# casys-kaist/CoVA

Hardware: AMD Instinct MI355X
Metric: compressed-domain frames/sec (BlobNet+bboxcc) at 1080p b=256 (higher is better)
Workload: dtype f16

## Files before the change

cova_amd/csrc/bboxcc.hip:

```cpp
#include <algorithm>
#include <cstdint>
#include <mutex>
#include <vector>

#include "bboxcc_body.h"
#include "bboxcc_wave.h"
#include "covahip_dev.h"
#include "internal.h"

namespace {

using namespace ccbody;

__global__ __launch_bounds__(CC_THREADS) void bboxcc_kernel(const uint8_t *__restrict__ masks, CcGeom g, ccwave::WvGeom wg,
                                                             int area_thresh, covahip_box *__restrict__ boxes,
                                                             int32_t *__restrict__ counts, int max_boxes,
                                                             const int32_t *__restrict__ list,
                                                             const int32_t *__restrict__ n_list,
                                                             const int32_t *__restrict__ stat_src, int32_t *__restrict__ stat_dst,
                                                             int stat_batch, int stat_cap) {
    extern __shared__ __attribute__((aligned(16))) uint8_t smem[];
    if (stat_dst && blockIdx.x == 0 && threadIdx.x < 8)
        stat_dst[threadIdx.x] = threadIdx.x < 5 ? stat_src[threadIdx.x] : threadIdx.x == 5 ? stat_batch : threadIdx.x == 6 ? stat_cap : 0;
    auto one = [&](int frame) {
// ... 32 lines not shown
                                                                    int area_thresh, covahip_box *__restrict__ boxes,
                                                                    int32_t *__restrict__ counts, int max_boxes,
                                                                    const int32_t *__restrict__ list, const int32_t *__restrict__ n_list,
                                                                    int32_t *__restrict__ ovf_list, int32_t *__restrict__ ovf_n,
                                                                    int base_cap, int32_t *__restrict__ n_big,
                                                                    int32_t *__restrict__ zero_next) {
    extern __shared__ __attribute__((aligned(16))) uint8_t smem[];
    const int lane = threadIdx.x & 63, wave = threadIdx.x >> 6;
    uint8_t *const sm = smem + (size_t)wave * g.wave_bytes;
    if constexpr (!LIST) {
        if (zero_next && blockIdx.x == 0 && threadIdx.x < 8) zero_next[threadIdx.x] = 0;
        const int frame = blockIdx.x * WV_WAVES + wave;
        if (frame >= batch) return;
        const int n = ccwave::frame_wave(masks + (size_t)frame * g.H * g.W, sm, g, area_thresh, boxes + (size_t)frame * max_boxes,
                                         counts + frame, max_boxes, lane);
        if (lane == 0) {
            if (n > g.cap) {
                const int k = atomicAdd(ovf_n, 1);
                if (k < batch) ovf_list[k] = frame;
            }
            if (n_big && (frame & 15) == 0 && n > base_cap)
                atomicAdd(n_big + (n > 2 * base_cap ? 2 : 2 * n > 3 * base_cap ? 1 : 0), 1);
        }
    } else {
        const int nl = min(*n_list, batch);
        for (int k = blockIdx.x * WV_WAVES + wave; k < nl; k += gridDim.x * WV_WAVES) {
            const int frame = list[k];
            const int n = ccwave::frame_wave(masks + (size_t)frame * g.H * g.W, sm, g, area_thresh, boxes + (size_t)frame * max_boxes,
                                             counts + frame, max_boxes, lane);
            if (lane == 0 && n > g.cap) {
                const int k2 = atomicAdd(ovf_n, 1);
                if (k2 < batch) ovf_list[k2] = frame;
            }
            ccwave::wave_fence();
        }
    }
}

template <typename K>
int open_lds(covahip_ctx *ctx, K kernel, size_t lds) {
    if (lds <= 64 * 1024) return COVAHIP_OK;
    static std::mutex mu;
    static std::vector<std::pair<int, const void *>> opened;
    const void *fn = reinterpret_cast<const void *>(kernel);
    std::lock_guard<std::mutex> lock(mu);
    for (auto &o : opened)
        if (o.first == ctx->device && o.second == fn) return COVAHIP_OK;
    COVAHIP_CHECK_HIP(ctx, hipFuncSetAttribute(fn, hipFuncAttributeMaxDynamicSharedMemorySize, 160 * 1024 - 64));
    opened.emplace_back(ctx->device, fn);
    return COVAHIP_OK;
}

}

constexpr int WAVE_CAP = 128;
int covahip_bboxcc_launch(covahip_ctx *ctx, const uint8_t *d_mask, int batch, int h, int w, int area_thresh,
                          covahip_box *d_boxes, int32_t *d_counts, int max_boxes) {
    if (batch == 0) return COVAHIP_OK;
    CtxLane &ln = ctx->lane();
    CcGeom g;
    const size_t lds = cc_plan(h, w, g);
    const int num_cu = ctx->props.multiProcessorCount;
    ccwave::WvGeom wg;
    const int nb = ((h + 1) / 2) * ((w + 1) / 2);
    int cap = ctx->cc_wave_cap;
    if (cap == 0) {
        cap = -1;
        if (batch > 3 * num_cu) {
            if (ln.cc_stat && ln.cc_stat[5] > 0) {
                const int64_t c1 = 16 * (int64_t)ln.cc_stat[2], c2 = 16 * (int64_t)ln.cc_stat[3], c3 = 16 * (int64_t)ln.cc_stat[4], sb = ln.cc_stat[5];
                ln.cc_first_cap = 4 * c3 > sb ? 4 * WAVE_CAP : 4 * (c2 + c3) > sb ? 2 * WAVE_CAP : 4 * (c1 + c2 + c3) > sb ? 3 * WAVE_CAP / 2 : WAVE_CAP;
            }
            cap = ln.cc_first_cap ? ln.cc_first_cap : WAVE_CAP;
        }
    }
    cap = std::min(cap, nb);
    const bool aligned = (reinterpret_cast<uintptr_t>(d_mask) & 7) == 0 && (((size_t)h * w) & 7) == 0;
    ccwave::WvGeom wfull{};
    size_t lds_wg = lds;
    if (ctx->cc_wave_cap >= 0 && aligned && ccwave::wv_plan(h, w, nb, wfull) && (size_t)wfull.wave_bytes <= 160 * 1024 - 256)
        lds_wg = (size_t)wfull.wave_bytes;
    else
        wfull.cap = 0;
    if (cap > 0 && aligned && ccwave::wv_plan(h, w, cap, wg) &&
        (size_t)WV_WAVES * wg.wave_bytes <= 160 * 1024 - 64 && (cap >= nb || lds_wg)) {
        const bool can_overflow = cap < nb;
        ccwave::WvGeom wg2{};
        const int cap2 = std::min(4 * cap, nb);
        const bool second = can_overflow && cap2 > cap && ccwave::wv_plan(h, w, cap2, wg2) &&
                            (size_t)WV_WAVES * wg2.wave_bytes <= 160 * 1024 - 64;
        const bool third = can_overflow && (!second || cap2 < nb);
        int32_t *ovf = nullptr;
        if (can_overflow) {
            const size_t need = (2 * (size_t)batch + 16) * sizeof(int32_t);
            const bool fresh = need > ln.cc_ovf_bytes;
            int rc = covahip_ensure_buffer(ctx, &ln.cc_ovf, &ln.cc_ovf_bytes, need);
            if (rc) return rc;
            if (fresh) {
                COVAHIP_CHECK_HIP(ctx, hipMemsetAsync(ln.cc_ovf, 0, 16 * sizeof(int32_t), ctx->stream));
                ln.cc_stat_turn = 0;
            }
            ovf = (int32_t *)ln.cc_ovf;
            if (!ln.cc_stat_ring) {
                COVAHIP_CHECK_HIP(ctx, hipHostMalloc((void **)&ln.cc_stat_ring, 8 * sizeof(int32_t), hipHostMallocMapped));
                for (int k = 0; k < 8; k++) ln.cc_stat_ring[k] = 0;
                ln.cc_stat = ln.cc_stat_ring;
            }
        }
        const unsigned set = can_overflow ? (ln.cc_stat_turn & 1) : 0;
        int32_t *cnt = ovf ? ovf + 8 * set : nullptr, *cnt_next = ovf ? ovf + 8 * (set ^ 1) : nullptr;
        int32_t *n1 = cnt, *n2 = cnt ? cnt + 1 : nullptr, *n_big = cnt ? cnt + 2 : nullptr;
        int32_t *list1 = ovf ? ovf + 16 : nullptr, *list2 = ovf ? ovf + 16 + batch : nullptr;
        const bool second_now = second && !(ln.cc_stat && ln.cc_stat[5] > 0 && ln.cc_stat[0] == 0);
        const size_t wlds = (size_t)WV_WAVES * wg.wave_bytes;
        int rc = open_lds(ctx, bboxcc_wave_kernel<false>, wlds);
        if (rc) return rc;
        if (second) rc = open_lds(ctx, bboxcc_wave_kernel<true>, (size_t)WV_WAVES * wg2.wave_bytes);
        if (rc) return rc;
        {
            ProfScope ps(ctx, "bboxcc_wave_kernel");
            hipLaunchKernelGGL(bboxcc_wave_kernel<false>, dim3((batch + WV_WAVES - 1) / WV_WAVES), dim3(WV_WAVES * 64), wlds, ctx->stream,
                               d_mask, wg, batch, area_thresh, d_boxes, d_counts, max_boxes, (const int32_t *)nullptr,
                               (const int32_t *)nullptr, list1, n1, WAVE_CAP, n_big, cnt_next);
            COVAHIP_CHECK_HIP(ctx, hipGetLastError());
            if (can_overflow) ln.cc_stat_turn++;
        }
        if (second_now) {
            const size_t wlds2 = (size_t)WV_WAVES * wg2.wave_bytes;
            const int per_cu = std::max(1, (int)((160 * 1024 - 256) / wlds2));
            const int grid = std::min((batch + WV_WAVES - 1) / WV_WAVES, per_cu * num_cu);
            ProfScope ps(ctx, "bboxcc_wave_kernel_2");
            hipLaunchKernelGGL(bboxcc_wave_kernel<true>, dim3(grid), dim3(WV_WAVES * 64), wlds2, ctx->stream, d_mask, wg2, batch, area_thresh,
                               d_boxes, d_counts, max_boxes, (const int32_t *)list1, (const int32_t *)n1, list2, n2, 0, (int32_t *)nullptr,
                               (int32_t *)nullptr);
            COVAHIP_CHECK_HIP(ctx, hipGetLastError());
        }
        if (can_overflow) {
            rc = open_lds(ctx, bboxcc_kernel, lds_wg);
            if (rc) return rc;
            int32_t *stat_dev = nullptr;
            COVAHIP_CHECK_HIP(ctx, hipHostGetDevicePointer((void **)&stat_dev, ln.cc_stat_ring, 0));
            const bool have_list = third || !second_now;
            const bool quiet = ln.cc_stat && ln.cc_stat[5] > 0 && ln.cc_stat[0] == 0;
            ProfScope ps(ctx, "bboxcc_kernel");
            hipLaunchKernelGGL(bboxcc_kernel, dim3(!have_list ? 1 : quiet ? 32 : std::min(batch, 2 * num_cu)), dim3(CC_THREADS), lds_wg, ctx->stream, d_mask, g, wfull,
                               area_thresh, d_boxes, d_counts, max_boxes, (const int32_t *)(second_now ? list2 : list1),
                               (const int32_t *)(second_now ? n2 : n1), (const int32_t *)cnt, stat_dev, batch, cap);
            COVAHIP_CHECK_HIP(ctx, hipGetLastError());
            ln.cc_stat_batch = batch;
            ln.cc_stat_cap = cap;
            ln.cc_second_skipped = !second_now;
        } else {
            ln.cc_stat_batch = 0;
        }
        return COVAHIP_OK;
    }
    ln.cc_stat_batch = 0;
    if (!lds_wg) {
        CcGeom gb;
        const size_t slab = cc_plan_global(h, w, gb);
        if (!slab) return COVAHIP_ERR_UNSUPPORTED;
        const int grid = std::min(batch, 2 * num_cu);
        int rc = covahip_ensure_buffer(ctx, &ln.cc_slab, &ln.cc_slab_bytes, slab * grid);
        if (rc) return rc;
        ProfScope ps(ctx, "bboxcc_big_kernel");
        hipLaunchKernelGGL(bboxcc_big_kernel, dim3(grid), dim3(CC_THREADS), 0, ctx->stream, d_mask, gb, (uint8_t *)ln.cc_slab, slab,
// ... 63 lines not shown
```

cova_amd/csrc/bboxcc_wave.h:

```cpp
#pragma once
#include <cstdint>

#include "bboxcc_body.h"

#ifdef PHASE_TIMING
__device__ unsigned long long g_ccph[8];
#define CCWG_MARK(i)                                                        \
    do {                                                                    \
        if (tid == 0) {                                                     \
            const unsigned long long now_ = __builtin_amdgcn_s_memrealtime(); \
            atomicAdd(&g_ccph[i], now_ - cc_last_);                         \
            cc_last_ = now_;                                                \
        }                                                                   \
    } while (0)
#else
#define CCWG_MARK(i) do { } while (0)
#endif

namespace ccwave {

struct WvGeom {
    int H, W, BH, BW, NXB;
    int cap;
    int rows_bytes;
    int wave_bytes;
    uint32_t mNXB;
};

inline bool wv_plan(int h, int w, int cap, WvGeom &g) {
    if (h <= 0 || w <= 0 || h > 128 || w > 128 || (w & 7) || cap <= 0) return false;
    g.H = h; g.W = w;
    g.BH = (h + 1) / 2; g.BW = (w + 1) / 2;
    g.NXB = w / 8;
    g.cap = cap;
    g.rows_bytes = (2 * g.BH + 2) * 16;
    g.wave_bytes = g.rows_bytes + cap * 24;
    g.mNXB = g.NXB <= 1 ? 0u : (uint32_t)(((1ull << 32) / (uint32_t)g.NXB) + 1);
    return true;
}

__device__ __forceinline__ uint32_t nz_bits(uint32_t x) {
    return (((x & 0x7F7F7F7Fu) + 0x7F7F7F7Fu) | x) & 0x80808080u;
}
__device__ __forceinline__ void wave_fence() {
    __builtin_amdgcn_fence(__ATOMIC_RELEASE, "wavefront");
    __builtin_amdgcn_wave_barrier();
    __builtin_amdgcn_fence(__ATOMIC_ACQUIRE, "wavefront");
}
__device__ __forceinline__ int ctz64(uint64_t x) { return __ffsll((unsigned long long)x) - 1; }
__device__ __forceinline__ int nth_set_bit64(uint64_t x, int k) {
    uint32_t w = (uint32_t)x;
    int pos = 0;
    int c = __popc(w);
    if (k >= c) { k -= c; w = (uint32_t)(x >> 32); pos = 32; }
    c = __popc(w & 0xFFFFu);
    if (k >= c) { k -= c; w >>= 16; pos += 16; }
    c = __popc(w & 0xFFu);
    if (k >= c) { k -= c; w >>= 8; pos += 8; }
    c = __popc(w & 0xFu);
    if (k >= c) { k -= c; w >>= 4; pos += 4; }
    w &= 0xFu;
    for (int i = 0; i < k; i++) w &= w - 1;
    return pos + (__ffs((int)w) - 1);
}
__device__ __forceinline__ uint64_t mask_upto(int e) { return e >= 63 ? ~0ull : ((2ull << e) - 1); }

__device__ __forceinline__ int frame_wave(const uint8_t *m, uint8_t *sm, const WvGeom &g, int area_thresh, covahip_box *ob,
                                           int32_t *count_out, int max_boxes, int lane) {
    uint32_t *rows = reinterpret_cast<uint32_t *>(sm);
    uint32_t *lab = reinterpret_cast<uint32_t *>(sm + g.rows_bytes);
    uint32_t *s_area = lab + g.cap, *s_minx = s_area + g.cap, *s_maxx = s_minx + g.cap, *s_miny = s_maxx + g.cap,
             *s_maxy = s_miny + g.cap;

    for (int i = lane; i < g.rows_bytes / 4; i += 64) rows[i] = 0;
    wave_fence();
    const int npieces = g.H * g.NXB;
    constexpr int UN = 8;
    for (int q0 = lane; q0 < npieces; q0 += 64 * UN) {
        uint2 v[UN];
#pragma unroll
        for (int k = 0; k < UN; k++) {
            const int q = q0 + 64 * k;
            v[k] = q < npieces ? *reinterpret_cast<const uint2 *>(m + (size_t)q * 8) : make_uint2(0, 0);
        }
#pragma unroll
        for (int k = 0; k < UN; k++) {
            if ((v[k].x | v[k].y) == 0) continue;
            const int q = q0 + 64 * k;
            const int y = g.mNXB ? (int)__umulhi((uint32_t)q, g.mNXB) : q, xc = q - y * g.NXB;
            const uint32_t tl = nz_bits(v[k].x), th = nz_bits(v[k].y);
            const uint32_t e = (((tl & 0x00800080u) * 0x00800100u) >> 30) | ((((th & 0x00800080u) * 0x00800100u) >> 30) << 2);
            const uint32_t o = (((tl & 0x80008000u) * 0x00008001u) >> 30) | ((((th & 0x80008000u) * 0x00008001u) >> 30) << 2);
            uint32_t *rw = rows + (y + 1) * 4 + (xc >> 3);
            const int sh = 4 * (xc & 7);
            if (e) atomicOr(rw, e << sh);
            if (o) atomicOr(rw + 2, o << sh);
        }
    }

    wave_fence();
    uint64_t a = 0, b = 0, c = 0, d = 0, ue = 0, uo = 0;
    if (lane < g.BH) {
        const uint4 ru = reinterpret_cast<const uint4 *>(rows)[2 * lane];
        const uint4 r0 = reinterpret_cast<const uint4 *>(rows)[2 * lane + 1];
        const uint4 r1 = reinterpret_cast<const uint4 *>(rows)[2 * lane + 2];
        ue = ru.x | ((uint64_t)ru.y << 32); uo = ru.z | ((uint64_t)ru.w << 32);
        a = r0.x | ((uint64_t)r0.y << 32);  b = r0.z | ((uint64_t)r0.w << 32);
        c = r1.x | ((uint64_t)r1.y << 32);  d = r1.z | ((uint64_t)r1.w << 32);
    }
    const uint64_t F = a | b | c | d;
    const uint64_t J = (a | c) & ((b | d) << 1);
    const uint64_t S = F & ~J;
// ... 77 lines not shown
    wave_fence();
    int total = 0;
    for (int i0 = 0; i0 < n; i0 += 64) {
        const int i = i0 + lane;
        const bool keep = i < n && lab[i] == (uint32_t)i && (int)s_area[i] >= area_thresh;
        const uint64_t bal = __ballot(keep);
        if (keep) {
            const int pos = total + __popcll((unsigned long long)(bal & ((1ull << lane) - 1)));
            if (pos < max_boxes) {
                covahip_box bx;
                bx.left = (int32_t)s_minx[i];
                bx.top = (int32_t)s_miny[i];
                bx.width = (int32_t)(s_maxx[i] - s_minx[i] + 1);
                bx.height = (int32_t)(s_maxy[i] - s_miny[i] + 1);
                bx.area_px = (int32_t)s_area[i];
                ob[pos] = bx;
            }
        }
        total += __popcll((unsigned long long)bal);
    }
    if (lane == 0) *count_out = total;
    return n;
}

template <int NTH, bool PLANES = false>
__device__ __forceinline__ void frame_wg(const uint8_t *m, uint8_t *sm, const WvGeom &g, int area_thresh, covahip_box *ob,
                                         int32_t *count_out, int max_boxes, int tid, uint32_t *planes = nullptr) {
    constexpr int NWV = NTH / 64;
    const int lane = tid & 63, wave = tid >> 6;
    uint32_t *rows = PLANES ? planes : reinterpret_cast<uint32_t *>(sm);
    uint32_t *lab = reinterpret_cast<uint32_t *>(sm + g.rows_bytes);
    uint32_t *s_area = lab + g.cap, *s_minx = s_area + g.cap, *s_maxx = s_minx + g.cap, *s_miny = s_maxx + g.cap,
             *s_maxy = s_miny + g.cap;
    __shared__ uint32_t wave_tot[NWV];
#ifdef PHASE_TIMING
    unsigned long long cc_last_ = __builtin_amdgcn_s_memrealtime();
#endif

    if constexpr (!PLANES) {
    for (int i = tid; i < g.rows_bytes / 4; i += NTH) rows[i] = 0;
    __syncthreads();
    const int npieces = g.H * g.NXB;
    for (int q = tid; q < npieces; q += NTH) {
        const uint2 v = *reinterpret_cast<const uint2 *>(__builtin_assume_aligned(m + (size_t)q * 8, 8));
        if ((v.x | v.y) == 0) continue;
        const int y = g.mNXB ? (int)__umulhi((uint32_t)q, g.mNXB) : q, xc = q - y * g.NXB;
        const uint32_t tl = nz_bits(v.x), th = nz_bits(v.y);
        const uint32_t e = (((tl & 0x00800080u) * 0x00800100u) >> 30) | ((((th & 0x00800080u) * 0x00800100u) >> 30) << 2);
        const uint32_t o = (((tl & 0x80008000u) * 0x00008001u) >> 30) | ((((th & 0x80008000u) * 0x00008001u) >> 30) << 2);
        uint32_t *rw = rows + (y + 1) * 4 + (xc >> 3);
        const int sh = 4 * (xc & 7);
        if (e) atomicOr(rw, e << sh);
        if (o) atomicOr(rw + 2, o << sh);
    }
    __syncthreads();
    }
    CCWG_MARK(0);
    uint64_t a = 0, b = 0, c = 0, d = 0, ue = 0, uo = 0;
    if (lane < g.BH) {
        const uint4 ru = reinterpret_cast<const uint4 *>(rows)[2 * lane];
        const uint4 r0 = reinterpret_cast<const uint4 *>(rows)[2 * lane + 1];
        const uint4 r1 = reinterpret_cast<const uint4 *>(rows)[2 * lane + 2];
        ue = ru.x | ((uint64_t)ru.y << 32); uo = ru.z | ((uint64_t)ru.w << 32);
        a = r0.x | ((uint64_t)r0.y << 32);  b = r0.z | ((uint64_t)r0.w << 32);
        c = r1.x | ((uint64_t)r1.y << 32);  d = r1.z | ((uint64_t)r1.w << 32);
    }
    const uint64_t F = a | b | c | d;
    const uint64_t J = (a | c) & ((b | d) << 1);
    const uint64_t S = F & ~J;
    const uint64_t cU = (a | b) & (ue | uo), cUL = a & (uo << 1), cUR = b & (ue >> 1);
    const int nr = __popcll((unsigned long long)S);
    int incl = nr;
#pragma unroll
    for (int o = 1; o < 64; o <<= 1) {
        const int t = __shfl_up(incl, o, 64);
        if (lane >= o) incl += t;
    }
    const int base = incl - nr;
    const int n = __shfl(incl, 63, 64);
    uint64_t S_up = (uint64_t)__shfl_up((unsigned long long)S, 1, 64), J_up = (uint64_t)__shfl_up((unsigned long long)J, 1, 64);
    int base_up = __shfl_up(base, 1, 64);
    if (lane == 0) { S_up = 0; J_up = 0; base_up = 0; }
    for (int i = tid; i < n; i += NTH) lab[i] = (uint32_t)i;
    __syncthreads();
    CCWG_MARK(1);
    for (int k = wave; __any(k < nr); k += NWV) {
        uint64_t Tu = 0;
        const int idx = base + k;
        if (k < nr) {
            const int s = nth_set_bit64(S, k);
            const uint64_t jr = (J >> s) >> 1;
            const int e = s + (~jr ? ctz64(~jr) : 0);
            const uint64_t mk = mask_upto(e) & ~((1ull << s) - 1);
            const uint64_t ra = a & mk, rb = b & mk, rc = c & mk, rd = d & mk;
            s_area[idx] = (uint32_t)(__popcll((unsigned long long)ra) + __popcll((unsigned long long)rb) +
                                     __popcll((unsigned long long)rc) + __popcll((unsigned long long)rd));
            s_minx[idx] = (uint32_t)(2 * s + (((a | c) >> s) & 1 ? 0 : 1));
            s_maxx[idx] = (uint32_t)(2 * e + (((b | d) >> e) & 1 ? 1 : 0));
            s_miny[idx] = (uint32_t)(2 * lane + ((ra | rb) ? 0 : 1));
            s_maxy[idx] = (uint32_t)(2 * lane + ((rc | rd) ? 1 : 0));
            Tu = (cU & mk) | ((cUL & mk) >> 1) | ((cUR & mk) << 1);
        }
        while (__any(Tu != 0)) {
            if (Tu) {
                const int p = ctz64(Tu);
                const int rank = __popcll((unsigned long long)(S_up << (63 - p))) - 1;
                const uint64_t jr = (J_up >> p) >> 1;
                const int e_up = p + (~jr ? ctz64(~jr) : 0);
                Tu &= ~mask_upto(e_up);
                ccbody::uf_union(lab, (uint32_t)idx, (uint32_t)(base_up + rank));
            }
        }
    }
    __syncthreads();
    CCWG_MARK(2);
    for (int i = tid; i < n; i += NTH) {
        const uint32_t root = ccbody::uf_find(lab, (uint32_t)i);
        if (root != (uint32_t)i) {
            lab[i] = root;
            atomicAdd(&s_area[root], s_area[i]);
            atomicMin(&s_minx[root], s_minx[i]);
            atomicMax(&s_maxx[root], s_maxx[i]);
            atomicMin(&s_miny[root], s_miny[i]);
            atomicMax(&s_maxy[root], s_maxy[i]);
        }
    }
    __syncthreads();
    CCWG_MARK(3);
    const int per = (n + NTH - 1) / NTH;
    const int i0 = tid * per;
    uint32_t cnt = 0;
    for (int k = 0; k < per; k++) {
        const int i = i0 + k;
        if (i < n && lab[i] == (uint32_t)i && (int)s_area[i] >= area_thresh) cnt++;
    }
    uint32_t inc2 = cnt;
#pragma unroll
    for (int o = 1; o < 64; o <<= 1) {
        const uint32_t t = __shfl_up(inc2, o, 64);
        if (lane >= o) inc2 += t;
    }
    if (lane == 63) wave_tot[wave] = inc2;
    __syncthreads();
    uint32_t pbase = 0, total = 0;
#pragma unroll
    for (int k = 0; k < NWV; k++) {
        const uint32_t t = wave_tot[k];
        if (k < wave) pbase += t;
        total += t;
    }
    uint32_t pos = pbase + inc2 - cnt;
    for (int k = 0; k < per; k++) {
        const int i = i0 + k;
        if (i < n && lab[i] == (uint32_t)i && (int)s_area[i] >= area_thresh) {
            if ((int)pos < max_boxes) {
                covahip_box bx;
                bx.left = (int32_t)s_minx[i];
                bx.top = (int32_t)s_miny[i];
                bx.width = (int32_t)(s_maxx[i] - s_minx[i] + 1);
                bx.height = (int32_t)(s_maxy[i] - s_miny[i] + 1);
                bx.area_px = (int32_t)s_area[i];
                ob[pos] = bx;
            }
            pos++;
        }
    }
    if (tid == 0) *count_out = (int32_t)total;
    __syncthreads();
// ... 5 lines not shown
```

cova_amd/csrc/blobnet.hip:

```cpp
#include <algorithm>
#include <cstdlib>
#include <cstring>
#include <vector>

#include "blobnet.h"
#include "covahip_dev.h"

namespace {

constexpr uint32_t W_MAGIC = 0x57485643;
constexpr size_t N_PARAMS = 320305;

}

static void free_model(covahip_ctx *ctx, covahip_blobnet *m) {
    if (!m) return;
    blobnet_release_mfma(ctx, m);
    for (BnWorkspace &ws : m->ws) {
        for (int i = 0; i <= BN_LEVELS; i++)
            if (ws.act[i]) hipFree(ws.act[i]);
        for (int j = 0; j < BN_LEVELS; j++)
            if (ws.dact[j]) hipFree(ws.dact[j]);
        if (ws.pbuf) hipFree(ws.pbuf);
        if (ws.part) hipFree(ws.part);
// ... 240 lines not shown
    BnInput plan;
    plan.dry = true;
    for (int pass = 0; pass < (n_models > 1 ? 8 : 4) && !rc; pass++) {
        const int b = (pass & 1) ? max_batch : 1;
        plan.n_frames = (pass & 2) ? b + BN_T - 1 : 0;
        plan.mixed = (pass & 4) != 0;
        rc = blobnet_forward_mfma(ctx, m, m->ws[0], plan, b, nullptr, nullptr, nullptr, nullptr);
    }
    return rc;
}

extern "C" {

static const float *check_blob(const void *weights, size_t weights_bytes) {
    if (!weights || weights_bytes < 64) return nullptr;
    uint32_t hdr[16];
    std::memcpy(hdr, weights, 64);
    static const uint32_t want[] = {W_MAGIC, 1, 4, 3, 16, 32, 64, 128, 64, 32, 16, 16, (uint32_t)N_PARAMS};
    for (int i = 0; i < 13; i++)
        if (hdr[i] != want[i]) return nullptr;
    if (weights_bytes != 64 + N_PARAMS * sizeof(float)) return nullptr;
    return reinterpret_cast<const float *>(static_cast<const uint8_t *>(weights) + 64);
}

int covahip_blobnet_load(covahip_ctx *ctx, const void *weights, size_t weights_bytes, int h_mb, int w_mb, int t,
                         int max_batch) {
    if (!ctx || !weights) return COVAHIP_ERR_INVALID_ARG;
    if (t == BN_T && h_mb >= 16 && w_mb >= 16 && h_mb <= 1024 && w_mb <= 1024 && max_batch > 0 && !check_blob(weights, weights_bytes))
        return COVAHIP_ERR_BAD_WEIGHTS;
    return covahip_blobnet_load_set(ctx, 1, &weights, &weights_bytes, h_mb, w_mb, t, max_batch);
}

int covahip_blobnet_load_set(covahip_ctx *ctx, int n_models, const void *const *weights, const size_t *weights_bytes, int h_mb,
                             int w_mb, int t, int max_batch) {
    if (!ctx || !weights || !weights_bytes || h_mb <= 0 || w_mb <= 0 || max_batch <= 0) return COVAHIP_ERR_INVALID_ARG;
    if (n_models < 1 || n_models > COVAHIP_MAX_MODELS) return COVAHIP_ERR_INVALID_ARG;
    for (int k = 0; k < n_models; k++)
        if (!weights[k]) return COVAHIP_ERR_INVALID_ARG;
    if (t != BN_T) return COVAHIP_ERR_UNSUPPORTED;
    if (h_mb < 16 || w_mb < 16 || h_mb > 1024 || w_mb > 1024) return COVAHIP_ERR_UNSUPPORTED;
    std::vector<const float *> h_w(n_models);
    bool bad = false;
    for (int k = 0; k < n_models; k++) bad = bad || !(h_w[k] = check_blob(weights[k], weights_bytes[k]));

    COVAHIP_CHECK_HIP(ctx, hipSetDevice(ctx->device));
    covahip_blobnet_destroy(ctx);
    if (bad) return COVAHIP_ERR_BAD_WEIGHTS;
    covahip_blobnet *m = new covahip_blobnet();
    int rc = build_model(ctx, m, h_w.data(), n_models, h_mb, w_mb, max_batch);
    if (rc == COVAHIP_OK && hipStreamSynchronize(ctx->stream) != hipSuccess) rc = COVAHIP_ERR_HIP;
    if (rc) {
        hipStreamSynchronize(ctx->stream);
        (void)hipGetLastError();
        free_model(ctx, m);
        return rc;
    }
    ctx->blobnet = m;
    return COVAHIP_OK;
}

int covahip_blobnet_num_models(covahip_ctx *ctx, int *n_models) {
    if (!ctx || !n_models) return COVAHIP_ERR_INVALID_ARG;
    if (!ctx->blobnet) return COVAHIP_ERR_NOT_LOADED;
    *n_models = ctx->blobnet->n_models;
    return COVAHIP_OK;
}

int covahip_blobnet_macs_per_frame(covahip_ctx *ctx, int64_t *macs) {
    if (!ctx || !macs) return COVAHIP_ERR_INVALID_ARG;
    if (!ctx->blobnet) return COVAHIP_ERR_NOT_LOADED;
    *macs = ctx->blobnet->macs_per_frame;
    return COVAHIP_OK;
}

int covahip_blobnet_set_enc_plan(covahip_ctx *ctx, int level, int nbands, int nbuf) {
    if (!ctx || level < 1 || level > 3 || nbands < 0 || nbands > 64 || (nbands && nbuf != 1 && nbuf != 2)) return COVAHIP_ERR_INVALID_ARG;
    ctx->enc_plan[level].nbands = nbands;
    ctx->enc_plan[level].nbuf = nbands ? nbuf : 0;
    return COVAHIP_OK;
}

int covahip_blobnet_set_impl(covahip_ctx *ctx, int impl) {
    if (!ctx || !ctx->blobnet) return COVAHIP_ERR_NOT_LOADED;
    if (impl != 1 && (impl < 4 || impl > 10)) return COVAHIP_ERR_INVALID_ARG;
    ctx->blobnet->fuse_dec = impl != 4;
    ctx->blobnet->enc1_tile16 = impl != 5;
    ctx->blobnet->enc_rowtiles = impl != 6;
    ctx->blobnet->fuse_enc23 = impl == 7 ? 0 : impl == 8 ? 2 : 1;
    ctx->blobnet->tail_part = impl != 9;
    ctx->blobnet->tail_rows = impl != 10;
    return COVAHIP_OK;
}

static int filter_placed(covahip_ctx *ctx, covahip_blobnet *m, const uint8_t *d_src, int n_frames, const int32_t *stack_index,
                         int batch, int area_thresh, covahip_box *d_boxes, int32_t *d_counts, int max_boxes, float *d_logits,
                         uint8_t *d_mask, bool packed = false, const uint8_t *model_ids = nullptr) {
    if (!d_mask) {
        CtxLane &l = ctx->lane();
        int rc = covahip_ensure_buffer(ctx, &l.cc_scratch, &l.cc_scratch_bytes, (size_t)batch * m->H * m->W);
        if (rc) return rc;
        d_mask = (uint8_t *)l.cc_scratch;
    }
    BnInput in;
    if (n_frames > 0) {
        int rc = prepare_frames(ctx, m, m->ws[ctx->cur_lane], d_src, n_frames, stack_index, batch, in, model_ids);
        if (rc) return rc;
        in.packed = packed;
    } else {
        in.stack = d_src;
    }
    return filter_dev(ctx, in, batch, d_logits, d_mask, true, area_thresh, d_boxes, d_counts, max_boxes, n_frames > 0 ? nullptr : model_ids);
}

static int filter_any(covahip_ctx *ctx, const uint8_t *src, int n_frames, const int32_t *stack_index, int batch,
                      int area_thresh, covahip_box *boxes, int32_t *counts, int max_boxes, float *logits, uint8_t *mask,
                      int mem_kind, const uint8_t *model_ids = nullptr) {
    if (!ctx || batch < 0 || max_boxes < 0 || n_frames < 0) return COVAHIP_ERR_INVALID_ARG;
    covahip_blobnet *m = ctx->blobnet;
    if (!m) return COVAHIP_ERR_NOT_LOADED;
    if (batch == 0) return COVAHIP_OK;
    if (!src || !counts || (!boxes && max_boxes > 0) || batch > m->max_batch) return COVAHIP_ERR_INVALID_ARG;
    if (int rc = check_model_ids(m, model_ids, batch)) return rc;
    COVAHIP_CHECK_HIP(ctx, hipSetDevice(ctx->device));
    const bool by_frames = n_frames > 0;
    const size_t hw = (size_t)m->H * m->W;
    const size_t in_bytes = by_frames ? (size_t)n_frames * hw * 4 : (size_t)batch * BN_T * hw * 4;
    const size_t mask_bytes = (size_t)batch * hw;
    const size_t logit_bytes = mask_bytes * sizeof(float);
    const size_t box_bytes = (size_t)batch * max_boxes * sizeof(covahip_box);
    const size_t cnt_bytes = (size_t)batch * sizeof(int32_t);
    auto al = [](size_t x) { return (x + 255) & ~(size_t)255; };
    if (mem_kind != COVAHIP_MEM_DEVICE && mem_kind != COVAHIP_MEM_HOST) return COVAHIP_ERR_INVALID_ARG;

    if (mem_kind == COVAHIP_MEM_DEVICE) {
        LaneScope lane(ctx);
        if (!lane.ok()) return COVAHIP_ERR_HIP;
        return filter_placed(ctx, m, src, n_frames, stack_index, batch, area_thresh, boxes, counts, max_boxes, logits, mask, false, model_ids);
    }
    if (int rc = covahip_primary_op(ctx)) return rc;
    const uint8_t *d_src = src;
    int rc = covahip_ensure_buffer(ctx, &ctx->stage_in, &ctx->stage_in_bytes, in_bytes);
    if (rc) return rc;
    rc = covahip_ensure_buffer(ctx, &ctx->stage_out, &ctx->stage_out_bytes,
                               al(mask_bytes) + al(logit_bytes) + al(box_bytes) + al(cnt_bytes));
    if (rc) return rc;
    uint8_t *base = (uint8_t *)ctx->stage_out;
    uint8_t *d_mask = base;
    float *d_logits = logits ? (float *)(base + al(mask_bytes)) : nullptr;
    covahip_box *d_boxes = (covahip_box *)(base + al(mask_bytes) + al(logit_bytes));
    int32_t *d_counts = (int32_t *)(base + al(mask_bytes) + al(logit_bytes) + al(box_bytes));
    COVAHIP_CHECK_HIP(ctx, hipMemcpyAsync(ctx->stage_in, src, in_bytes, hipMemcpyHostToDevice, ctx->stream));
    d_src = (const uint8_t *)ctx->stage_in;
    rc = filter_placed(ctx, m, d_src, n_frames, stack_index, batch, area_thresh, d_boxes, d_counts, max_boxes, d_logits, d_mask, false,
                       model_ids);
    if (rc) return rc;
    if (logits) COVAHIP_CHECK_HIP(ctx, hipMemcpyAsync(logits, d_logits, logit_bytes, hipMemcpyDeviceToHost, ctx->stream));
    if (mask) COVAHIP_CHECK_HIP(ctx, hipMemcpyAsync(mask, d_mask, mask_bytes, hipMemcpyDeviceToHost, ctx->stream));
    if (box_bytes) COVAHIP_CHECK_HIP(ctx, hipMemcpyAsync(boxes, d_boxes, box_bytes, hipMemcpyDeviceToHost, ctx->stream));
    COVAHIP_CHECK_HIP(ctx, hipMemcpyAsync(counts, d_counts, cnt_bytes, hipMemcpyDeviceToHost, ctx->stream));
    COVAHIP_CHECK_HIP(ctx, hipStreamSynchronize(ctx->stream));
    return COVAHIP_OK;
}

int covahip_filter_forward(covahip_ctx *ctx, const uint8_t *rgba_stack, int batch, int area_thresh,
                           covahip_box *boxes, int32_t *counts, int max_boxes, float *logits, uint8_t *mask,
                           int mem_kind) {
    return filter_any(ctx, rgba_stack, 0, nullptr, batch, area_thresh, boxes, counts, max_boxes, logits, mask, mem_kind);
}

int covahip_filter_forward_m(covahip_ctx *ctx, const uint8_t *rgba_stack, const uint8_t *model_ids, int batch, int area_thresh,
                             covahip_box *boxes, int32_t *counts, int max_boxes, float *logits, uint8_t *mask, int mem_kind) {
    return filter_any(ctx, rgba_stack, 0, nullptr, batch, area_thresh, boxes, counts, max_boxes, logits, mask, mem_kind, model_ids);
}
// ... 169 lines not shown
```

cova_amd/csrc/blobnet_mfma.hip:

```cpp
#include <algorithm>
#include <cmath>
#include <cstdlib>
#include <cstring>
#include <mutex>
#include <type_traits>
#include <utility>
#include <vector>

#include "bboxcc_body.h"
#include "bboxcc_wave.h"
#include "blobnet.h"

typedef _Float16 half8 __attribute__((ext_vector_type(8)));
typedef _Float16 half4 __attribute__((ext_vector_type(4)));
typedef float f32x16 __attribute__((ext_vector_type(16)));
typedef float f32x4 __attribute__((ext_vector_type(4)));
typedef _Float16 half2v __attribute__((ext_vector_type(2)));

namespace {

constexpr float BN_EPS = 1e-3f;
constexpr int WG = 256;

struct EncPrep {
// ... 2688 lines not shown
    return true;
}

struct DecPlan {
    DecArgs a;
    DecMs am;
    BnLevelGeom in, out;
    bool half;
    int ci, GH, grid;
    size_t row_bytes, lds;
};
int plan_dec_block(const Fwd &f, int j, DecPlan &p) {
    const covahip_blobnet *m = f.m;
    const Prepared *pr = f.pr;
    const BnLevelGeom in = m->lv[BN_LEVELS - j], out = m->lv[BN_LEVELS - 1 - j];
    const bool last = j == BN_LEVELS - 1;
    const bool half = last && f.part_written;
    const int ci_j = half ? m->dec_ci[j] / 2 : m->dec_ci[j];
    DecArgs &a = p.a;
    a.up = j == 0 ? nullptr : f.ws.dact[j - 1];
    a.skip = f.ws.act[BN_LEVELS - j];
    a.out = last ? nullptr : f.ws.dact[j];
    a.logits = last ? f.d_logits : nullptr;
    a.mask = last ? f.d_mask : nullptr;
    a.wfrag = (const half8 *)(f.prep + (half ? pr->final_w_up : last ? pr->final_w : pr->dec[j].wfrag));
    a.part = half ? f.ws.part : nullptr;
    a.epi = (const float *)(f.prep + (last ? pr->final_epi : pr->dec[j].epi));
    a.B = f.batch; a.Hi = in.H; a.Wi = in.W; a.Hd = out.H; a.Wd = out.W; a.cy = m->dec_cy[j]; a.cx = m->dec_cx[j];
    a.Ts = j == 0 ? 1 : BN_T;
    p.am = DecMs{f.inp.model_ids, f.mstride};
    const int GH = in.H + 1;
    const size_t row_bytes = (size_t)(in.W + 2) * ci_j * 2;
    const size_t wbytes = (size_t)(last ? 1 : 4 * m->dec_co[j] / 32) * (4 * ci_j / 16) * 1024;
    const bool heavy = wbytes >= 192 * 1024 && (size_t)(GH + 1) * row_bytes <= 72 * 1024;
    int nbands = 1;
    if (!heavy)
        while (nbands < GH && (((size_t)((GH + nbands - 1) / nbands) + 1) * row_bytes > 30 * 1024 ||
                               (long long)f.batch * nbands < 2LL * f.num_cu))
            nbands++;
    a.nbands = nbands; a.mNb = magic(nbands); a.mGW = magic(in.W + 1);
    a.mRC = magic((in.W + 2) * (ci_j / 8)); a.zero = f.prep + pr->zero;
    a.swz = choose_swz(false, ci_j, in.W, 0, (GH + nbands - 1) / nbands);
    const size_t tile_bytes = (((size_t)((GH + nbands - 1) / nbands) + 1) * row_bytes + 15) & ~(size_t)15;
    const size_t mask_bytes = last ? ((((size_t)2 * ((GH + nbands - 1) / nbands) * out.W) + 15) & ~(size_t)15) : 0;
    const size_t scr_bytes = last ? 0 : (size_t)std::max(4, 4 * m->dec_co[j] / 32) * 2048;
    p.lds = tile_bytes + mask_bytes + scr_bytes;
    a.mask_off = (int)tile_bytes;
    a.scr_off = (int)tile_bytes;
    if (p.lds > 160 * 1024 - 256) return COVAHIP_ERR_UNSUPPORTED;
    p.in = in; p.out = out; p.half = half; p.ci = ci_j; p.GH = GH; p.row_bytes = row_bytes;
    p.grid = std::min(f.batch * nbands, (heavy ? 1 : 4) * f.num_cu);
    return COVAHIP_OK;
}
int launch_dec_block(const Fwd &f, int j, const DecPlan &p) {
    if (j == 0)
        return launched(f, with_bools([&](auto MS) {
            return launch(f, "dec0_mfma", dec_mfma<0, 128, 64, false, MS.value>, p.grid, 512, p.lds, p.a, p.am);
        }, f.ms));
    if (j == 1)
        return launched(f, with_bools([&](auto MS) {
            return launch(f, "dec1_mfma", dec_mfma<64, 64, 32, false, MS.value>, p.grid, 256, p.lds, p.a, p.am);
        }, f.ms));
    if (j == 2)
        return launched(f, with_bools([&](auto MS) {
            return launch(f, "dec2_mfma", dec_mfma<32, 32, 16, false, MS.value>, p.grid, 256, p.lds, p.a, p.am);
        }, f.ms));
    return launched(f, with_bools([&](auto HALF, auto MS) {
        return launch(f, "dec3_final_mfma", dec_mfma<16, HALF.value ? 0 : 16, 16, true, MS.value>, p.grid, 256, p.lds, p.a, p.am);
    }, p.half, f.ms));
}
int run_dec_block(const Fwd &f, int j) {
    DecPlan p;
    if (int rc = plan_dec_block(f, j, p)) return rc;
    return launch_dec_block(f, j, p);
}

bool run_tail_fused(const Fwd &f, const DecPlan &p) {
    const BnLevelGeom in = p.in, out = p.out;
    const int GH = p.GH;
    Dec3ccArgs t;
    size_t cc_bytes = ccbody::cc_plan(out.H, out.W, t.g);
    t.use_wv = f.ctx->cc_wave_cap >= 0 && ccwave::wv_plan(out.H, out.W, ((out.H + 1) / 2) * ((out.W + 1) / 2), t.wg) ? 1 : 0;
    if (t.use_wv) cc_bytes = (size_t)t.wg.wave_bytes;
    if (!cc_bytes) return false;
    const size_t mfull = ((size_t)out.H * out.W + 15) & ~(size_t)15;
    const size_t partb = p.half ? (size_t)GH * (in.W + 1) * 16 : 0;
    int best_nb = 0;
    long long best_cost = -1;
    for (int nb = 1; nb <= GH; nb++) {
        const size_t tb = (((size_t)((GH + nb - 1) / nb) + 1) * p.row_bytes + 15) & ~(size_t)15;
        const size_t nbuf = nb == 1 ? 1 : 2;
        if (std::max(nbuf * tb, cc_bytes) + mfull + partb > 160 * 1024 - 512) continue;
        long long rounds = 0;
        for (int k = 0; k < nb; k++) {
            const int nu = (k + 1) * GH / nb - k * GH / nb;
            rounds += ((nu * (in.W + 1) + 31) / 32 + 15) / 16;
        }
        const long long cost = rounds * 8 + nb;
        if (best_cost < 0 || cost < best_cost) { best_cost = cost; best_nb = nb; }
    }
    if (!best_nb) return false;
    const size_t tb = (((size_t)((GH + best_nb - 1) / best_nb) + 1) * p.row_bytes + 15) & ~(size_t)15;
    t.d = p.a;
    t.ms = p.am;
    t.d.nbands = best_nb; t.d.mNb = magic(best_nb);
    t.d.swz = choose_swz(false, p.ci, in.W, 0, (GH + best_nb - 1) / best_nb);
    t.boxes = f.cc->boxes; t.counts = f.cc->counts;
    t.area_thresh = f.cc->area_thresh; t.max_boxes = f.cc->max_boxes;
    t.tile_bytes = (int)tb; t.cc_off = 0;
    t.mfull_off = (int)std::max((best_nb == 1 ? 1 : 2) * tb, cc_bytes);
    t.part_off = (int)((size_t)t.mfull_off + mfull);
    const size_t tl = (size_t)t.part_off + partb;
    const int grid = std::min(f.batch, 2 * f.num_cu);
    if (p.half && t.use_wv && best_nb == 1 && in.W + 1 <= 64 && f.m->tail_rows && (out.W & 7) == 0 &&
        (size_t)t.wg.rows_bytes <= mfull && (!f.d_mask || (reinterpret_cast<uintptr_t>(f.d_mask) & 3) == 0)) {
        t.d.swz = Swz{3, 1, 0, 0, 0};
        t.d.mRC = magic(out.W / 4);
        return !with_bools([&](auto MS) {
            return launch(f, "dec3_bboxcc_fused", dec3cc_rows_mfma<MS.value>, grid, ccbody::CC_THREADS, tl, t);
        }, f.ms);
    }
    return !with_bools([&](auto WV, auto PART, auto MS) {
        return launch(f, "dec3_bboxcc_fused", dec3cc_mfma<WV.value, PART.value, MS.value>, grid, ccbody::CC_THREADS, tl, t);
    }, t.use_wv != 0, p.half, f.ms);
}

}

int blobnet_forward_mfma(covahip_ctx *ctx, covahip_blobnet *m, BnWorkspace &ws, const BnInput &inp, int batch, float *d_logits,
                         uint8_t *d_mask, const BnCcTail *cc, bool *cc_done) {
    if (cc_done) *cc_done = false;
    const Prepared *pr = m->prep;
    const bool dry = inp.dry;
    const bool by_frames = inp.frames != nullptr || (dry && inp.n_frames > 0);
    const bool ms = inp.model_ids != nullptr || (dry && inp.mixed);
    Fwd f{ctx, m, pr, ws, inp, batch,
          (const uint8_t *)m->d_prepared + (ms ? 0 : (size_t)inp.model * pr->total), (uint32_t)pr->total,
          ms, dry, by_frames, ctx->props.multiProcessorCount,
          by_frames ? inp.frames : inp.stack, by_frames ? inp.n_frames : batch * BN_T, by_frames ? inp.index : nullptr,
          d_logits, d_mask, cc};
    if ((size_t)f.n_frames > ws.pbuf_frames && !dry) return COVAHIP_ERR_INVALID_ARG;

    int rc = run_enc0p(f);
    if (rc) return rc;
    if (!run_enc1_tile16(f, rc)) rc = run_enc_level(f, 1);
    if (rc) return rc;
    if (!run_enc23(f, rc)) {
        rc = run_enc_level(f, 2);
        if (!rc) rc = run_enc_level(f, 3);
    }
    if (rc) return rc;
    if (!run_dec012(f, rc))
        for (int j = 0; j < BN_LEVELS - 1 && !rc; j++) rc = run_dec_block(f, j);
    if (rc) return rc;
    DecPlan last;
    rc = plan_dec_block(f, BN_LEVELS - 1, last);
    if (rc) return rc;
    if (!(cc && m->fuse_tail && run_tail_fused(f, last))) return launch_dec_block(f, BN_LEVELS - 1, last);
    if (cc_done) *cc_done = true;
    return launched(f, COVAHIP_OK);
}

#if defined(PHASE_TIMING) || defined(WGSPAN_ONLY)
extern "C" int covahip_dev_wgspan_read(unsigned long long *out, int kid) {
    return hipMemcpyFromSymbol(out, HIP_SYMBOL(g_wgspan), sizeof(unsigned long long) * 1024 * 4, sizeof(unsigned long long) * 1024 * 4 * kid) != hipSuccess;
}
// ... 25 lines not shown
```

cova_amd/csrc/internal.h:

```cpp
#pragma once
#include <hip/hip_runtime.h>

#include <cstdint>
#include <map>
#include <string>
#include <vector>

#include "covahip.h"

struct covahip_blobnet;

constexpr int COVAHIP_MAX_LANES = 4;
struct CtxLane {
    hipStream_t stream = nullptr;
    hipEvent_t done = nullptr;
    bool pending = false;
    uint64_t seen_seq = 0;
    void *cc_scratch = nullptr;
    size_t cc_scratch_bytes = 0;
    void *cc_ovf = nullptr;
    size_t cc_ovf_bytes = 0;
    void *cc_slab = nullptr;
    size_t cc_slab_bytes = 0;
    int32_t *cc_stat = nullptr;
    int32_t *cc_stat_ring = nullptr;
    unsigned cc_stat_turn = 0;
    bool cc_second_skipped = false;
    int cc_stat_batch = 0, cc_stat_cap = 0;
    int cc_first_cap = 0;
};

struct covahip_ctx {
    int device = 0;
    hipStream_t primary = nullptr;
    hipStream_t stream = nullptr;
    CtxLane lanes[COVAHIP_MAX_LANES];
    int n_lanes = 1, next_lane = 0, cur_lane = 0;
    bool in_lane = false;
    uint64_t primary_seq = 1;
    hipEvent_t ev_fork = nullptr;
    std::string last_hip_error;
    hipDeviceProp_t props{};
    hipEvent_t t_start[16]{};
    hipEvent_t t_stop[16]{};
    bool profile = false;
    std::string profile_filter;
    struct ProfEntry {
        std::string name;
        hipEvent_t a, b;
    };
    std::vector<ProfEntry> prof_pending;
    std::vector<std::pair<hipEvent_t, hipEvent_t>> prof_pool;
    std::map<std::string, std::pair<double, int64_t>> prof_acc;
    void *stage_in = nullptr;
    size_t stage_in_bytes = 0;
    void *stage_out = nullptr;
    size_t stage_out_bytes = 0;
    void *pinned = nullptr;
    size_t pinned_bytes = 0;
    int cc_wave_cap = 0;
    CtxLane &lane() { return lanes[cur_lane]; }
    struct { int nbands, nbuf; } enc_plan[4] = {};
    covahip_blobnet *blobnet = nullptr;
};

#define COVAHIP_CHECK_HIP(ctx, expr)                                                        \
    do {                                                                                    \
        hipError_t _e = (expr);                                                             \
        if (_e != hipSuccess) {                                                             \
            (ctx)->last_hip_error = std::string(#expr) + ": " + hipGetErrorString(_e);      \
            return COVAHIP_ERR_HIP;                                                         \
        }                                                                                   \
    } while (0)

struct ProfScope {
    covahip_ctx *ctx;
    int idx = -1;
    ProfScope(covahip_ctx *c, const char *name);
    ~ProfScope();
};

int covahip_ensure_buffer(covahip_ctx *ctx, void **buf, size_t *cur, size_t need);

struct LaneScope {
    covahip_ctx *ctx;
    bool owner = false, failed = false;
    explicit LaneScope(covahip_ctx *c);
    ~LaneScope();
    bool ok() const { return !failed; }
};
int covahip_primary_op(covahip_ctx *ctx);
int covahip_sync_all(covahip_ctx *ctx);

uint32_t covahip_crc32c(const uint8_t *p, size_t n);

int covahip_bboxcc_launch(covahip_ctx *ctx, const uint8_t *d_mask, int batch, int h, int w, int area_thresh,
                          covahip_box *d_boxes, int32_t *d_counts, int max_boxes);

void covahip_blobnet_destroy(covahip_ctx *ctx);
int covahip_blobnet_forward_dev(covahip_ctx *ctx, const uint8_t *d_stack, int batch, float *d_logits,
                                uint8_t *d_mask, const uint8_t *model_ids = nullptr);
int covahip_blobnet_geometry(covahip_ctx *ctx, int *h, int *w);
int covahip_blobnet_grow_lanes(covahip_ctx *ctx, int n_lanes);
```

cova_amd/elements.py:

```python
from __future__ import annotations

import ctypes as C

import numpy as np

from . import _lib as L
from . import weights as W

FLOW_OK = "ok"
FLOW_DROPPED = "dropped"


def _ptr(a: np.ndarray) -> int:
    return a.ctypes.data


def _optr(a: np.ndarray | None) -> int | None:
    return None if a is None else a.ctypes.data


class Context:

    def __init__(self, device_id: int = 0):
        self._lib = L.lib()
# ... 58 lines not shown
        ms = C.c_float()
        L.check(self._lib.covahip_timer_elapsed_ms(self.handle, slot, C.byref(ms)), "timer_elapsed", self.handle)
        return ms.value

    def profile(self, on: bool, only: str | None = None):
        L.check(self._lib.covahip_profile_filter(self.handle, only.encode() if only else None), "profile_filter")
        L.check(self._lib.covahip_profile_enable(self.handle, int(on)), "profile_enable")
        L.check(self._lib.covahip_profile_reset(self.handle), "profile_reset")

    def profile_read(self):
        buf = np.zeros(64, dtype=L.KERNEL_TIME_DTYPE)
        n = C.c_int()
        L.check(self._lib.covahip_profile_read(self.handle, _ptr(buf), 64, C.byref(n)), "profile_read")
        return {r["name"].decode(): (float(r["total_ms"]), int(r["launches"])) for r in buf[:n.value]}


class MetaPreprocess:

    def __init__(self, timestep: int = 1, gamma: int = 1):
        self.timestep = timestep
        self.gamma = gamma
        self._h = None
        self._lib = L.lib()

    def transform_caps(self, width: int, height: int):
        ow, oh = C.c_int(), C.c_int()
        self._lib.covahip_stack_out_dims(width, height, self.timestep, C.byref(ow), C.byref(oh))
        return ow.value, oh.value

    def set_caps(self, width: int, height: int):
        ow, oh = self.transform_caps(width, height)
        out_size = ow * oh * 4
        self.size_per_buf = out_size // self.timestep
        self.out_size = out_size
        self.stop()
        h = C.c_void_p()
        L.check(self._lib.covahip_stack_new(self.size_per_buf, self.timestep, self.gamma, C.byref(h)), "stack_new")
        self._h = h
        return ow, oh

    def transform(self, inbuf: bytes | np.ndarray):
        a = np.frombuffer(inbuf, dtype=np.uint8) if not isinstance(inbuf, np.ndarray) else inbuf.reshape(-1)
        a = np.ascontiguousarray(a, dtype=np.uint8)
        out = np.empty(self.out_size, dtype=np.uint8)
        em = C.c_int()
        L.check(self._lib.covahip_stack_push(self._h, _ptr(a), a.size, _ptr(out), out.size, C.byref(em)), "stack_push")
        return (FLOW_OK, out) if em.value else (FLOW_DROPPED, None)

    def stop(self):
        if self._h:
            self._lib.covahip_stack_free(self._h)
            self._h = None

    __del__ = stop


class BlobNetInfer:

    def __init__(self, ctx: Context, weights_flat, h_mb: int, w_mb: int, max_batch: int,
                 timestep: int = 4):
        self.ctx, self.h, self.w, self.t, self.max_batch = ctx, h_mb, w_mb, timestep, max_batch
        self._lib = L.lib()
        if isinstance(weights_flat, (list, tuple)):
            blobs = [W.to_bytes(w) for w in weights_flat]
            ptrs = (C.c_char_p * max(1, len(blobs)))(*blobs)
            sizes = (C.c_size_t * max(1, len(blobs)))(*[len(b) for b in blobs])
            L.check(self._lib.covahip_blobnet_load_set(ctx.handle, len(blobs), ptrs, sizes, h_mb, w_mb, timestep, max_batch),
                    "covahip_blobnet_load_set", ctx.handle)
        else:
            blob = W.to_bytes(weights_flat)
            L.check(self._lib.covahip_blobnet_load(ctx.handle, blob, len(blob), h_mb, w_mb, timestep, max_batch),
                    "covahip_blobnet_load", ctx.handle)

    @property
    def num_models(self) -> int:
        v = C.c_int()
        L.check(self._lib.covahip_blobnet_num_models(self.ctx.handle, C.byref(v)), "covahip_blobnet_num_models")
        return v.value

    def set_enc_plan(self, level: int, nbands: int, nbuf: int = 1):
        L.check(self._lib.covahip_blobnet_set_enc_plan(self.ctx.handle, level, nbands, nbuf), "covahip_blobnet_set_enc_plan")

    def set_impl(self, impl: str):
        L.check(self._lib.covahip_blobnet_set_impl(self.ctx.handle, {"mfma": 1, "dec_separate": 4, "enc1_legacy": 5, "enc_general_tiles": 6, "enc23_separate": 7, "enc23_force": 8, "tail_skip_tensor": 9, "tail_band_tiles": 10}[impl]), "set_impl")

    def read_buffer(self, which: int, index: int = 0) -> np.ndarray:
        p, n, dims = C.c_void_p(), C.c_size_t(), (C.c_int32 * 5)()
        L.check(self._lib.covahip_dev_blobnet_buffer(self.ctx.handle, which, index, C.byref(p), C.byref(n), dims),
                "covahip_dev_blobnet_buffer", self.ctx.handle)
        out = np.empty(tuple(d for d in dims if d), dtype=np.float32 if which == 3 else np.float16)
        assert p.value and out.nbytes == n.value, (which, index, n.value, tuple(dims))
        self.ctx.d2h(out, p.value)
        return out

    @property
    def macs_per_frame(self) -> int:
        v = C.c_int64()
        L.check(self._lib.covahip_blobnet_macs_per_frame(self.ctx.handle, C.byref(v)), "macs_per_frame")
        return v.value

    def infer(self, stack: np.ndarray, want_logits: bool = True, model_ids=None):
        stack = np.ascontiguousarray(stack, dtype=np.uint8)
        b = stack.shape[0]
        assert stack.shape == (b, self.t * self.h, self.w, 4), stack.shape
        logits = np.empty((b, self.h, self.w), dtype=np.float32) if want_logits else None
        mask = np.empty((b, self.h, self.w), dtype=np.uint8)
        ids = _ids(model_ids, b)
        L.check(self._lib.covahip_blobnet_forward_m(self.ctx.handle, _ptr(stack), _optr(ids), b, _ptr(logits) if want_logits else None,
                                                    _ptr(mask), L.MEM_HOST), "covahip_blobnet_forward_m", self.ctx.handle)
        return logits, mask

    def infer_device(self, d_stack: int, batch: int, d_logits: int | None, d_mask: int | None, model_ids=None):
        ids = _ids(model_ids, batch)
        L.check(self._lib.covahip_blobnet_forward_m(self.ctx.handle, d_stack, _optr(ids), batch, d_logits, d_mask, L.MEM_DEVICE),
                "covahip_blobnet_forward_m", self.ctx.handle)

    def filter(self, stack: np.ndarray, cc_threshold: int, max_boxes: int = 256, want_mask: bool = False, model_ids=None):
        return self.filter_full(stack, cc_threshold, max_boxes, want_mask, False, model_ids)[:3]

    def filter_full(self, stack: np.ndarray, cc_threshold: int, max_boxes: int = 256, want_mask: bool = False,
                    want_logits: bool = False, model_ids=None):
        stack = np.ascontiguousarray(stack, dtype=np.uint8)
        b = stack.shape[0]
        boxes = np.zeros((b, max_boxes), dtype=L.BOX_DTYPE)
        counts = np.zeros(b, dtype=np.int32)
        mask = np.empty((b, self.h, self.w), dtype=np.uint8) if want_mask else None
        logits = np.empty((b, self.h, self.w), dtype=np.float32) if want_logits else None
        ids = _ids(model_ids, b)
        L.check(self._lib.covahip_filter_forward_m(self.ctx.handle, _ptr(stack), _optr(ids), b, cc_threshold, _ptr(boxes), _ptr(counts),
                                                   max_boxes, _ptr(logits) if want_logits else None, _ptr(mask) if want_mask else None,
                                                   L.MEM_HOST),
                "covahip_filter_forward_m", self.ctx.handle)
        return boxes, counts, mask, logits

    def filter_frames(self, frames: np.ndarray, stack_index: np.ndarray | None, cc_threshold: int, max_boxes: int = 256,
                      want_mask: bool = False, want_logits: bool = False, model_ids=None):
        frames = np.ascontiguousarray(frames, dtype=np.uint8)
        f = frames.shape[0]
        assert frames.shape == (f, self.h, self.w, 4), frames.shape
        idx = None if stack_index is None else np.ascontiguousarray(stack_index, dtype=np.int32).reshape(-1, 4)
        b = f - 3 if idx is None else idx.shape[0]
        boxes = np.zeros((b, max_boxes), dtype=L.BOX_DTYPE)
        counts = np.zeros(b, dtype=np.int32)
        mask = np.empty((b, self.h, self.w), dtype=np.uint8) if want_mask else None
        logits = np.empty((b, self.h, self.w), dtype=np.float32) if want_logits else None
        ids = _ids(model_ids, b)
        L.check(self._lib.covahip_filter_forward_frames_m(self.ctx.handle, _ptr(frames), f, None if idx is None else _ptr(idx),
                                                          _optr(ids), b, cc_threshold, _ptr(boxes), _ptr(counts), max_boxes,
                                                          _ptr(logits) if want_logits else None,
                                                          _ptr(mask) if want_mask else None, L.MEM_HOST),
                "covahip_filter_forward_frames_m", self.ctx.handle)
        return boxes, counts, mask, logits

    def filter_frames_device(self, d_frames: int, n_frames: int, stack_index: np.ndarray | None, batch: int, cc_threshold: int,
                             d_boxes: int, d_counts: int, max_boxes: int, d_mask: int | None = None, model_ids=None,
                             d_logits: int | None = None, packed: bool = False):
        idx = None if stack_index is None else np.ascontiguousarray(stack_index, dtype=np.int32).reshape(-1, 4)
        ids = _ids(model_ids, batch)
        if packed:
            L.check(self._lib.covahip_filter_forward_frames_packed_m(self.ctx.handle, d_frames, n_frames, None if idx is None else _ptr(idx),
                                                                     _optr(ids), batch, cc_threshold, d_boxes, d_counts, max_boxes,
                                                                     d_logits, d_mask),
                    "covahip_filter_forward_frames_packed_m", self.ctx.handle)
            return
        L.check(self._lib.covahip_filter_forward_frames_m(self.ctx.handle, d_frames, n_frames, None if idx is None else _ptr(idx),
                                                          _optr(ids), batch, cc_threshold, d_boxes, d_counts, max_boxes, d_logits,
                                                          d_mask, L.MEM_DEVICE),
# ... 435 lines not shown
```

Before: 2.371 million.

## Parallelize bboxcc run processing across threads instead of per-row wave lanes

Adds a new default path in the wave-level connected-components kernel. Each thread first scatters (row, start bit, upper-row base) records for every run into LDS. Threads then process runs in a flat thread-per-run loop, recomputing run extents and unions from the row bitmasks in LDS. The previous row-per-lane loop, kept behind a cc_row_lanes impl switch, could leave lanes idle when rows had uneven run counts. The new path costs an extra scatter pass, more LDS reads, and packs fields into s_minx, which assumes rows fit in 8 bits.

Measured after the change: 2.370 million. About the same (-0.0%).

```diff
diff --git a/cova_amd/csrc/bboxcc.hip b/cova_amd/csrc/bboxcc.hip
--- a/cova_amd/csrc/bboxcc.hip
+++ b/cova_amd/csrc/bboxcc.hip
@@ -138,6 +138,7 @@
         lds_wg = (size_t)wfull.wave_bytes;
     else
         wfull.cap = 0;
+    wfull.row_lanes = ctx->cc_row_lanes;
     if (cap > 0 && aligned && ccwave::wv_plan(h, w, cap, wg) &&
         (size_t)WV_WAVES * wg.wave_bytes <= 160 * 1024 - 64 && (cap >= nb || lds_wg)) {
         const bool can_overflow = cap < nb;
diff --git a/cova_amd/csrc/bboxcc_wave.h b/cova_amd/csrc/bboxcc_wave.h
--- a/cova_amd/csrc/bboxcc_wave.h
+++ b/cova_amd/csrc/bboxcc_wave.h
@@ -25,9 +25,11 @@
     int rows_bytes;
     int wave_bytes;
     uint32_t mNXB;
+    int row_lanes;
 };
 
 inline bool wv_plan(int h, int w, int cap, WvGeom &g) {
+    g.row_lanes = 0;
     if (h <= 0 || w <= 0 || h > 128 || w > 128 || (w & 7) || cap <= 0) return false;
     g.H = h; g.W = w;
     g.BH = (h + 1) / 2; g.BW = (w + 1) / 2;
@@ -271,8 +273,61 @@
     int base_up = __shfl_up(base, 1, 64);
     if (lane == 0) { S_up = 0; J_up = 0; base_up = 0; }
     for (int i = tid; i < n; i += NTH) lab[i] = (uint32_t)i;
+    if (!g.row_lanes) {
+        for (int u0 = 0; u0 < 16 * g.BH; u0 += NTH) {
+            const int u = u0 + tid, r = u >> 4, q4 = 4 * (u & 15);
+            const uint64_t Sr = (uint64_t)__shfl((unsigned long long)S, r & 63, 64);
+            const int br = __shfl(base, r & 63, 64), bu = __shfl(base_up, r & 63, 64);
+            uint32_t nib = r < g.BH ? (uint32_t)(Sr >> q4) & 15u : 0u;
+            if (nib) {
+                int idx = br + __popcll((unsigned long long)(Sr & ((1ull << q4) - 1)));
+                do {
+                    s_minx[idx++] = (uint32_t)(bu << 16 | r << 8 | (q4 + __ffs((int)nib) - 1));
+                    nib &= nib - 1;
+                } while (nib);
+            }
+        }
+    }
     __syncthreads();
     CCWG_MARK(1);
+    if (!g.row_lanes)
+    for (int i = tid; i < n; i += NTH) {
+        const uint32_t rs = s_minx[i];
+        const int r = (int)(rs >> 8) & 63, s = (int)(rs & 63u);
+        const uint4 qu = reinterpret_cast<const uint4 *>(rows)[2 * r];
+        const uint4 q0 = reinterpret_cast<const uint4 *>(rows)[2 * r + 1];
+        const uint4 q1 = reinterpret_cast<const uint4 *>(rows)[2 * r + 2];
+        const uint64_t pe = qu.x | ((uint64_t)qu.y << 32), po = qu.z | ((uint64_t)qu.w << 32);
+        const uint64_t pa = q0.x | ((uint64_t)q0.y << 32), pb = q0.z | ((uint64_t)q0.w << 32);
+        const uint64_t pc = q1.x | ((uint64_t)q1.y << 32), pd = q1.z | ((uint64_t)q1.w << 32);
+        const uint64_t jr = (((pa | pc) & ((pb | pd) << 1)) >> s) >> 1;
+        const int e = s + (~jr ? ctz64(~jr) : 0);
+        const uint64_t mk = mask_upto(e) & ~((1ull << s) - 1);
+        const uint64_t ra = pa & mk, rb = pb & mk, rc = pc & mk, rd = pd & mk;
+        s_area[i] = (uint32_t)(__popcll((unsigned long long)ra) + __popcll((unsigned long long)rb) +
+                               __popcll((unsigned long long)rc) + __popcll((unsigned long long)rd));
+        s_minx[i] = (uint32_t)(2 * s + (((pa | pc) >> s) & 1 ? 0 : 1));
+        s_maxx[i] = (uint32_t)(2 * e + (((pb | pd) >> e) & 1 ? 1 : 0));
+        s_miny[i] = (uint32_t)(2 * r + ((ra | rb) ? 0 : 1));
+        s_maxy[i] = (uint32_t)(2 * r + ((rc | rd) ? 1 : 0));
+        uint64_t Tu = ((ra | rb) & (pe | po)) | ((ra & (po << 1)) >> 1) | ((rb & (pe >> 1)) << 1);
+        if (Tu) {
+            const uint4 qt = reinterpret_cast<const uint4 *>(rows)[max(2 * r - 1, 0)];
+            const uint64_t ta = qt.x | ((uint64_t)qt.y << 32), tb = qt.z | ((uint64_t)qt.w << 32);
+            const uint64_t Ju = (ta | pe) & ((tb | po) << 1);
+            const uint64_t Su = (ta | tb | pe | po) & ~Ju;
+            const uint32_t bu = rs >> 16;
+            do {
+                const int p = ctz64(Tu);
+                const int rank = __popcll((unsigned long long)(Su << (63 - p))) - 1;
+                const uint64_t ju = (Ju >> p) >> 1;
+                const int e_up = p + (~ju ? ctz64(~ju) : 0);
+                Tu &= ~mask_upto(e_up);
+                ccbody::uf_union(lab, (uint32_t)i, bu + (uint32_t)rank);
+            } while (Tu);
+        }
+    }
+    else
     for (int k = wave; __any(k < nr); k += NWV) {
         uint64_t Tu = 0;
         const int idx = base + k;
diff --git a/cova_amd/csrc/blobnet.hip b/cova_amd/csrc/blobnet.hip
--- a/cova_amd/csrc/blobnet.hip
+++ b/cova_amd/csrc/blobnet.hip
@@ -346,13 +346,14 @@
 
 int covahip_blobnet_set_impl(covahip_ctx *ctx, int impl) {
     if (!ctx || !ctx->blobnet) return COVAHIP_ERR_NOT_LOADED;
-    if (impl != 1 && (impl < 4 || impl > 10)) return COVAHIP_ERR_INVALID_ARG;
+    if (impl != 1 && (impl < 4 || impl > 11)) return COVAHIP_ERR_INVALID_ARG;
     ctx->blobnet->fuse_dec = impl != 4;
     ctx->blobnet->enc1_tile16 = impl != 5;
     ctx->blobnet->enc_rowtiles = impl != 6;
     ctx->blobnet->fuse_enc23 = impl == 7 ? 0 : impl == 8 ? 2 : 1;
     ctx->blobnet->tail_part = impl != 9;
     ctx->blobnet->tail_rows = impl != 10;
+    ctx->cc_row_lanes = impl == 11;
     return COVAHIP_OK;
 }
 
diff --git a/cova_amd/csrc/blobnet_mfma.hip b/cova_amd/csrc/blobnet_mfma.hip
--- a/cova_amd/csrc/blobnet_mfma.hip
+++ b/cova_amd/csrc/blobnet_mfma.hip
@@ -2794,6 +2794,7 @@
     size_t cc_bytes = ccbody::cc_plan(out.H, out.W, t.g);
     t.use_wv = f.ctx->cc_wave_cap >= 0 && ccwave::wv_plan(out.H, out.W, ((out.H + 1) / 2) * ((out.W + 1) / 2), t.wg) ? 1 : 0;
     if (t.use_wv) cc_bytes = (size_t)t.wg.wave_bytes;
+    t.wg.row_lanes = f.ctx->cc_row_lanes;
     if (!cc_bytes) return false;
     const size_t mfull = ((size_t)out.H * out.W + 15) & ~(size_t)15;
     const size_t partb = p.half ? (size_t)GH * (in.W + 1) * 16 : 0;
diff --git a/cova_amd/csrc/internal.h b/cova_amd/csrc/internal.h
--- a/cova_amd/csrc/internal.h
+++ b/cova_amd/csrc/internal.h
@@ -59,6 +59,7 @@
     void *pinned = nullptr;
     size_t pinned_bytes = 0;
     int cc_wave_cap = 0;
+    int cc_row_lanes = 0;
     CtxLane &lane() { return lanes[cur_lane]; }
     struct { int nbands, nbuf; } enc_plan[4] = {};
     covahip_blobnet *blobnet = nullptr;
diff --git a/cova_amd/elements.py b/cova_amd/elements.py
--- a/cova_amd/elements.py
+++ b/cova_amd/elements.py
@@ -164,7 +164,7 @@
         L.check(self._lib.covahip_blobnet_set_enc_plan(self.ctx.handle, level, nbands, nbuf), "covahip_blobnet_set_enc_plan")
 
     def set_impl(self, impl: str):
-        L.check(self._lib.covahip_blobnet_set_impl(self.ctx.handle, {"mfma": 1, "dec_separate": 4, "enc1_legacy": 5, "enc_general_tiles": 6, "enc23_separate": 7, "enc23_force": 8, "tail_skip_tensor": 9, "tail_band_tiles": 10}[impl]), "set_impl")
+        L.check(self._lib.covahip_blobnet_set_impl(self.ctx.handle, {"mfma": 1, "dec_separate": 4, "enc1_legacy": 5, "enc_general_tiles": 6, "enc23_separate": 7, "enc23_force": 8, "tail_skip_tensor": 9, "tail_band_tiles": 10, "cc_row_lanes": 11}[impl]), "set_impl")
 
     def read_buffer(self, which: int, index: int = 0) -> np.ndarray:
         p, n, dims = C.c_void_p(), C.c_size_t(), (C.c_int32 * 5)()
```
